# emtiyaz/vmp-for-svae

Measured on AMD Instinct MI355X. Metric: vmp_step_datapoints_per_sec, higher is better.
Workload: dtype f32

## Files before the change

vmp-for-svae_amd/csrc/vmp_mix.hip:

```cpp
#include "vmp_common.h"
#include <stdlib.h>
#include <type_traits>

using namespace vmp;

namespace {

constexpr int TR = 64;
constexpr int LS = 68;
constexpr int MAX_NW = 8;
constexpr int MAX_NW1 = 8;
constexpr int max_nw(int KT) { return KT == 1 ? MAX_NW1 : MAX_NW; }
constexpr int MAX_BLOCKS = 1024;

struct PassArgs {
    const float* x;
    const float* r_in;
    const float* u_in;
    const uint8_t* mask;
    const float* pivot;
    const float* pack;
    float* r_out;
    float* u_out;
    float* logr_out;
    double* partials;
    long long N;
    long long rpw;
    long long rpw_b;
    int K;
    int vec_ok;
    int par_reduce;
#ifdef VMP_DEBUG_TS
    long long* dbg_t;
#endif
};
#ifdef VMP_DEBUG_TS
#define PASS_TS(i) do { if (a.dbg_t && (blockIdx.x == 0 || blockIdx.x == 100) && (threadIdx.x & 63) == 0) { a.dbg_t[(blockIdx.x ? 64 : 0) + (threadIdx.x >> 6) * 8 + (i)] = clock64(); \
    if ((i) == 0 && threadIdx.x == 0) a.dbg_t[(blockIdx.x ? 64 : 0) + 7] = wall_clock64();           \
    if ((i) == 5 && threadIdx.x == 64) a.dbg_t[(blockIdx.x ? 64 : 0) + 8 + 7] = wall_clock64(); } } while (0)
#else
#define PASS_TS(i) do { } while (0)
#endif

template <int D>
__device__ __forceinline__ void load_row(const float* __restrict__ p, float (&o)[D], bool vec) {
    if constexpr (D % 4 == 0) {
        if (vec) {
#pragma unroll
            for (int j = 0; j < D / 4; ++j) {
                float4 v = reinterpret_cast<const float4*>(p)[j];
                o[4 * j] = v.x; o[4 * j + 1] = v.y; o[4 * j + 2] = v.z; o[4 * j + 3] = v.w;
            }
            return;
        }
    } else if constexpr (D % 2 == 0) {
        if (vec) {
#pragma unroll
            for (int j = 0; j < D / 2; ++j) {
                float2 v = reinterpret_cast<const float2*>(p)[j];
                o[2 * j] = v.x; o[2 * j + 1] = v.y;
            }
            return;
        }
    }
#pragma unroll
    for (int j = 0; j < D; ++j) o[j] = p[j];
}

#define VMP_DPP2(OP, CTRL)                                                   \
    "v_" OP "_f32_dpp %0, %0, %0 " CTRL " row_mask:0xf bank_mask:0xf\n\t"  \
    "v_" OP "_f32_dpp %1, %1, %1 " CTRL " row_mask:0xf bank_mask:0xf\n\t"  \
    "s_nop 0\n\t"
#define VMP_DPP2_FIRST(OP, CTRL)                                             \
    "v_" OP "_f32_dpp %0, %2, %2 " CTRL " row_mask:0xf bank_mask:0xf\n\t"  \
    "v_" OP "_f32_dpp %1, %3, %3 " CTRL " row_mask:0xf bank_mask:0xf\n\t"  \
    "s_nop 0\n\t"
__device__ __forceinline__ v2f row16_max2(v2f v) {
    float a, b;
    asm("s_nop 1\n\t" VMP_DPP2_FIRST("max", "row_ror:8") VMP_DPP2("max", "row_ror:4") VMP_DPP2("max", "row_ror:2")
        VMP_DPP2("max", "row_ror:1")
        : "=&v"(a), "=&v"(b) : "v"(v.x), "v"(v.y));
    return v2f{a, b};
}
__device__ __forceinline__ v2f row16_sum2(v2f v) {
    float a, b;
    asm("s_nop 1\n\t" VMP_DPP2_FIRST("add", "row_ror:8") VMP_DPP2("add", "row_ror:4") VMP_DPP2("add", "row_ror:2")
        VMP_DPP2("add", "row_ror:1")
        : "=&v"(a), "=&v"(b) : "v"(v.x), "v"(v.y));
    return v2f{a, b};
}

constexpr int MOM_TERMS = 3;
#ifndef VMP_MOM_FLUSH
#define VMP_MOM_FLUSH 2
#endif

__device__ __forceinline__ double readlane_d(double v, int src_lane) {
    int lo = __double2loint(v), hi = __double2hiint(v);
    lo = __builtin_amdgcn_readlane(lo, src_lane);
    hi = __builtin_amdgcn_readlane(hi, src_lane);
    return __hiloint2double(hi, lo);
}

template <int D, int KT, int FLAV>
__device__ __forceinline__ void pass_epilogue(const PassArgs& a, float* smem, const double (&dacc)[KT][Geo<D>::FT][4],
                                              const double (&dn)[KT][4], int lane, int wave, int nw) {
    using G = Geo<D>;
    constexpr int FT = G::FT;
    constexpr bool SMM = (FLAV == VMP_SMM);
    const int K = a.K;
    {
        __syncthreads();
        PASS_TS(3);
        double* sc = reinterpret_cast<double*>(smem);
        constexpr int SLAB = KT * (FT + 1) * 4 * WAVE;
        if (a.par_reduce) {
            double* mine = sc + wave * SLAB;
#pragma unroll
            for (int kt = 0; kt < KT; ++kt)
#pragma unroll
                for (int c = 0; c < 4; ++c) {
#pragma unroll
                    for (int ft = 0; ft < FT; ++ft) mine[((kt * (FT + 1) + ft) * 4 + c) * WAVE + lane] = dacc[kt][ft][c];
                    mine[((kt * (FT + 1) + FT) * 4 + c) * WAVE + lane] = SMM ? dn[kt][c] : dacc[kt][0][c];
                }
            __syncthreads();
            constexpr int EPT = 2, NWB = max_nw(KT);
            for (int e0 = threadIdx.x; e0 < SLAB; e0 += EPT * blockDim.x) {
                double vals[EPT][NWB];
#pragma unroll
                for (int q = 0; q < EPT; ++q) {
                    const int e = e0 + q * blockDim.x;
#pragma unroll
                    for (int w = 0; w < NWB; ++w) vals[q][w] = (e < SLAB && w < nw) ? sc[w * SLAB + e] : 0.0;
                }
#pragma unroll
                for (int q = 0; q < EPT; ++q) {
                    const int e = e0 + q * blockDim.x;
                    double t2 = vals[q][0];
#pragma unroll
                    for (int w = 1; w < NWB; ++w) t2 += vals[q][w];
                    if (e < SLAB) sc[e] = t2;
                }
            }
            __syncthreads();
        } else {
            for (int w = 0; w < nw; ++w) {
                if (wave == w) {
#pragma unroll
                    for (int kt = 0; kt < KT; ++kt)
#pragma unroll
                        for (int c = 0; c < 4; ++c) {
#pragma unroll
                            for (int ft = 0; ft < FT; ++ft) {
                                const int idx = ((kt * (FT + 1) + ft) * 4 + c) * WAVE + lane;
                                sc[idx] = (w == 0 ? 0.0 : sc[idx]) + dacc[kt][ft][c];
                            }
                            const int idn = ((kt * (FT + 1) + FT) * 4 + c) * WAVE + lane;
                            sc[idn] = (w == 0 ? 0.0 : sc[idn]) + (SMM ? dn[kt][c] : dacc[kt][0][c]);
                        }
                }
                __syncthreads();
            }
        }
        PASS_TS(4);
        constexpr int PX = G::PF + 1;
        double* out = a.partials;
        for (int e = threadIdx.x; e < KT * (FT + 1) * 4 * WAVE; e += blockDim.x) {
            const int l = e & 63, c = (e >> 6) & 3, tf = (e >> 8) % (FT + 1), kt = (e >> 8) / (FT + 1);
            const int k = kt * 16 + (l >> 4) * 4 + c;
            if (k >= K) continue;
            double* row = out + ((long long)k * MAX_BLOCKS + blockIdx.x) * PX;
            if (tf < FT) {
                const int f = tf * 16 + (l & 15);
                if (f < G::F) row[f] = sc[e];
            } else if ((l & 15) == 0) {
                row[G::F] = sc[e];
            }
        }
        if (wave == 0) {
            double ntot = 0.0;
#pragma unroll
            for (int kt = 0; kt < KT; ++kt) {
                const int k = kt * 16 + (lane & 15), l = ((k & 15) >> 2) * 16, c = k & 3;
                const double nk = (lane < 16 && k < K) ? sc[((kt * (FT + 1) + FT) * 4 + c) * WAVE + l] : 0.0;
#pragma unroll
                for (int j = 0; j < 16; ++j) ntot += readlane_d(nk, j);
            }
            for (int k = lane; k < K; k += WAVE) out[((long long)k * MAX_BLOCKS + blockIdx.x) * PX + G::PF] = ntot;
        }
        PASS_TS(5);
    }
}

template <int D, int KT, int FLAV, bool ESTEP, bool STATS, bool MASK>
__global__ __launch_bounds__(max_nw(KT) * WAVE) void pass_kernel(PassArgs a) {
    using G = Geo<D>;
    constexpr int FT = G::FT;
    constexpr bool SMM = (FLAV == VMP_SMM);
    extern __shared__ __attribute__((aligned(16))) float smem[];

    const int lane = threadIdx.x & 63, wave = threadIdx.x >> 6, nw = blockDim.x >> 6;
    const int K = a.K;
    PASS_TS(0);
#ifdef VMP_DEBUG_TS
    if (a.dbg_t && (blockIdx.x == 0 || blockIdx.x == 100) && (threadIdx.x & 63) == 0)
        a.dbg_t[(blockIdx.x ? 64 : 0) + (threadIdx.x >> 6) * 8 + 6] = __builtin_amdgcn_s_getreg((31 << 11) | 4);
#endif
    float* xl = smem + wave * (G::XROWS * LS);
    constexpr int ONE = D, ZERO = D + 1;
    xl[ONE * LS + lane] = 1.0f;
    xl[ZERO * LS + lane] = 0.0f;
    const int ppos = (lane & ~7) + 2 * (lane & 3) + ((lane >> 2) & 1);

    const bool vec = a.vec_ok != 0;
    long long lo, hi;
    if (a.rpw_b == a.rpw) {
        lo = ((long long)blockIdx.x * nw + wave) * a.rpw;
        hi = lo + a.rpw;
    } else {
        const int hw = nw >> 1;
        const long long base = (long long)blockIdx.x * hw * (a.rpw + a.rpw_b);
        lo = wave < hw ? base + wave * a.rpw : base + hw * a.rpw + (wave - hw) * a.rpw_b;
        hi = lo + (wave < hw ? a.rpw : a.rpw_b);
    }
    if (hi > a.N) hi = a.N;
    float xr[D];
    {
        const long long n = lo + lane;
#pragma unroll
        for (int j = 0; j < D; ++j) xr[j] = 0.f;
        if (n < hi) load_row<D>(a.x + n * D, xr, vec);
    }
    const int i16 = lane & 15, kk = lane >> 4;
    float pv[D];
    {
        const float* __restrict__ pp = a.pivot ? a.pivot : a.x;
        const bool hasp = a.pivot != nullptr;
#pragma unroll
        for (int j = 0; j < D; ++j) { const float v = pp[j]; pv[j] = hasp ? v : 0.f; }
    }

    constexpr int MP = (D + 1) / 2, WP = (G::TRI + 1) / 2;
    v2f pm2[KT][MP], pw2[KT][WP], pch[KT];
    float pua[KT], pub[KT];
    if constexpr (ESTEP) {
#pragma unroll
        for (int kt = 0; kt < KT; ++kt) {
            const int k = kt * 16 + i16;
            const bool on = k < K;
            const float* __restrict__ p = a.pack + (on ? k : 0) * G::PACK;
            float raw[G::PACK];
            if (G::PACK % 4 == 0 && (reinterpret_cast<uintptr_t>(a.pack) & 15) == 0) {
#pragma unroll
                for (int j = 0; j < G::PACK / 4; ++j) {
                    const float4 q = reinterpret_cast<const float4*>(p)[j];
                    raw[4 * j] = q.x; raw[4 * j + 1] = q.y; raw[4 * j + 2] = q.z; raw[4 * j + 3] = q.w;
                }
            } else {
#pragma unroll
                for (int j = 0; j < G::PACK; ++j) raw[j] = p[j];
            }
#pragma unroll
            for (int j = 0; j < 2 * MP; ++j) pm2[kt][j >> 1][j & 1] = (on && j < D) ? raw[j < D ? j : 0] - pv[j < D ? j : 0] : 0.f;
#pragma unroll
            for (int j = 0; j < 2 * WP; ++j) pw2[kt][j >> 1][j & 1] = (on && j < G::TRI) ? raw[D + (j < G::TRI ? j : 0)] : 0.f;
            pch[kt].x = on ? raw[D + G::TRI] : -INFINITY;
            pch[kt].y = on ? raw[D + G::TRI + 1] : 0.f;
            pua[kt] = on ? raw[D + G::TRI + 2] : 0.f;
            pub[kt] = on ? raw[D + G::TRI + 3] : 1.f;
        }
    }

    int offA[FT], offB[FT];
#pragma unroll
    for (int ft = 0; ft < FT; ++ft) {
        const int f = ft * 16 + i16;
        int ra = ZERO, rb = ZERO;
        if (f == 0) { ra = ONE; rb = ONE; }
        else if (f <= D) { ra = f - 1; rb = ONE; }
        else if (f < G::F) {
            int p = f - D - 1, d = 0;
            while (p >= D - d) { p -= D - d; ++d; }
            ra = d; rb = d + p;
        }
        offA[ft] = ra * LS + 2 * kk;
        offB[ft] = rb * LS + 2 * kk;
    }

    f32x4 acc[KT][FT], acs[KT][FT];
    f32x4 nacc[KT], nacs[KT];
    double dacc[KT][FT][4];
    double dn[KT][4];
#pragma unroll
    for (int kt = 0; kt < KT; ++kt) {
        nacc[kt] = f32x4{0.f, 0.f, 0.f, 0.f};
        nacs[kt] = f32x4{0.f, 0.f, 0.f, 0.f};
#pragma unroll
        for (int c = 0; c < 4; ++c) dn[kt][c] = 0.0;
#pragma unroll
        for (int ft = 0; ft < FT; ++ft) {
            acc[kt][ft] = f32x4{0.f, 0.f, 0.f, 0.f};
            acs[kt][ft] = f32x4{0.f, 0.f, 0.f, 0.f};
#pragma unroll
            for (int c = 0; c < 4; ++c) dacc[kt][ft][c] = 0.0;
        }
    }

#ifdef VMP_DEBUG_TS
    if (a.dbg_t) {
        float chk = xr[0] + pv[0];
        if constexpr (ESTEP) chk += pm2[0][0][0] + pch[0].x;
        asm volatile("" :: "v"(chk));
        PASS_TS(1);
    }
#endif
    for (long long row0 = lo; row0 < hi; row0 += TR) {
        const int trows = (hi - row0 < TR) ? (int)(hi - row0) : TR;
        {
            const bool valid = row0 + lane < hi;
#pragma unroll
            for (int j = 0; j < D; ++j) xl[j * LS + ppos] = valid ? xr[j] - pv[j] : 0.f;
            const long long n2 = row0 + TR + lane;
#pragma unroll
            for (int j = 0; j < D; ++j) xr[j] = 0.f;
            if (n2 < hi) load_row<D>(a.x + n2 * D, xr, vec);
        }
        __builtin_amdgcn_wave_barrier();

        const long long tbase = (row0 + kk) * K + i16;
        const int K4 = 4 * K;
#pragma unroll 1
        for (int n0 = 0; n0 < trows; n0 += 32) {
            unsigned As[KT][3][4], Rs[KT][3][4], Bs[FT][3][4];
            auto group = [&](auto full_c, auto u_c) __attribute__((always_inline)) {
                constexpr bool FULL = decltype(full_c)::value;
                constexpr int u = decltype(u_c)::value;
                const int n8 = n0 + 8 * u;
// ... 549 lines not shown
                for (int ft = 0; ft < FT; ++ft)
#pragma unroll
                    for (int t = 0; t < 3; ++t)
                        b[ft][t] = __builtin_bit_cast(bf16x8, u32x4{Bs[ft][t][0], Bs[ft][t][1], Bs[ft][t][2], Bs[ft][t][3]});
                bf16x8 av[3];
#pragma unroll
                for (int t = 0; t < 3; ++t) av[t] = __builtin_bit_cast(bf16x8, u32x4{As[t][0], As[t][1], As[t][2], As[t][3]});
#pragma unroll
                for (int ta = 0; ta < MT; ++ta) {
#pragma unroll
                    for (int tb = 0; tb + ta < MT; ++tb) {
#pragma unroll
                        for (int ft = 0; ft < FT; ++ft) {
                            if (ta + tb == 0) acc[0][ft] = __builtin_amdgcn_mfma_f32_16x16x32_bf16(av[ta], b[ft][tb], acc[0][ft], 0, 0, 0);
                            else acs[0][ft] = __builtin_amdgcn_mfma_f32_16x16x32_bf16(av[ta], b[ft][tb], acs[0][ft], 0, 0, 0);
                        }
                    }
                }
            }
            };
            if (full) body(std::integral_constant<bool, true>{});
            else body(std::integral_constant<bool, false>{});
        }

        if constexpr (STATS) {
            if (((row0 - lo) / TR) % VMP_MOM_FLUSH == VMP_MOM_FLUSH - 1 || row0 + TR >= hi) {
#pragma unroll
                for (int c = 0; c < 4; ++c) {
#pragma unroll
                    for (int ft = 0; ft < FT; ++ft) dacc[0][ft][c] += (double)acc[0][ft][c] + (double)acs[0][ft][c];
                }
                if constexpr (SMM) { dnl += (double)nsum; nsum = 0.f; }
#pragma unroll
                for (int ft = 0; ft < FT; ++ft) { acc[0][ft] = f32x4{0.f, 0.f, 0.f, 0.f}; acs[0][ft] = f32x4{0.f, 0.f, 0.f, 0.f}; }
            }
        }
        __builtin_amdgcn_wave_barrier();
    }

    PASS_TS(2);
    if constexpr (STATS && SMM) {
        double tot = dnl;
        {
            int lo = __double2loint(tot), hi = __double2hiint(tot);
            tot += __hiloint2double(__shfl_xor(hi, 32), __shfl_xor(lo, 32));
            lo = __double2loint(tot); hi = __double2hiint(tot);
            tot += __hiloint2double(__shfl_xor(hi, 16), __shfl_xor(lo, 16));
        }
#pragma unroll
        for (int c = 0; c < 4; ++c) {
            const int src = 4 * kk + c;
            const int lo = __shfl(__double2loint(tot), src), hi = __shfl(__double2hiint(tot), src);
            dn[0][c] = __hiloint2double(hi, lo);
        }
    }
    if constexpr (STATS) pass_epilogue<D, 1, FLAV>(a, smem, dacc, dn, lane, wave, nw);
}

template <int D, int FLAV, bool STATS, int MT = 3>
__global__ __launch_bounds__(MAX_NW1 * WAVE) void pass_xdl_kernel(PassArgs a) {
    pass_xdl_body<D, FLAV, STATS, MT>(a);
}

__device__ double digamma_d(double x) {
    double r = 0.0;
    while (x < 10.0) { r -= 1.0 / x; x += 1.0; }
    const double f = 1.0 / (x * x);
    return r + log(x) - 0.5 / x
           - f * (1.0 / 12 - f * (1.0 / 120 - f * (1.0 / 252 - f * (1.0 / 240 - f * (1.0 / 132 - f * (691.0 / 32760))))));
}

template <int D>
__device__ void write_pack(float* pack, int k, const double* m, const double* W ,
                           double c, double h, double ua, double ub) {
    using G = Geo<D>;
    float* p = pack + k * G::PACK;
    int idx = D;
    for (int j = 0; j < D; ++j) p[j] = (float)m[j];
    for (int i = 0; i < D; ++i)
        for (int j = 0; j <= i; ++j) p[idx++] = (float)W[i * D + j];
    const double LOG2E = 1.4426950408889634074;
    p[idx++] = (float)(c * LOG2E); p[idx++] = (float)(h * LOG2E); p[idx++] = (float)ua; p[idx++] = (float)ub;
}

template <int D>
__device__ __forceinline__ bool chol_lower(double (&A)[D * D]) {
    bool ok = true;
#pragma unroll
    for (int j = 0; j < D; ++j) {
        double s = A[j * D + j];
#pragma unroll
        for (int p = 0; p < j; ++p) s -= A[j * D + p] * A[j * D + p];
        ok = ok && (s > 0.0);
        const double d = sqrt(s);
        const double rd = 1.0 / d;
        A[j * D + j] = d;
#pragma unroll
        for (int i = j + 1; i < D; ++i) {
            double t = A[i * D + j];
#pragma unroll
            for (int p = 0; p < j; ++p) t -= A[i * D + p] * A[j * D + p];
            A[i * D + j] = t * rd;
        }
#pragma unroll
        for (int i = 0; i < j; ++i) A[i * D + j] = 0.0;
    }
    return ok;
}

template <int D>
__device__ __forceinline__ void tri_inv_lower(const double (&L)[D * D], double (&Li)[D * D]) {
#pragma unroll
    for (int i = 0; i < D * D; ++i) Li[i] = 0.0;
#pragma unroll
    for (int j = 0; j < D; ++j) {
        Li[j * D + j] = 1.0 / L[j * D + j];
#pragma unroll
        for (int i = j + 1; i < D; ++i) {
            double s = 0.0;
#pragma unroll
            for (int p = j; p < i; ++p) s += L[i * D + p] * Li[p * D + j];
            Li[i * D + j] = -s / L[i * D + i];
        }
    }
}



__device__ __forceinline__ double fast_rsqrt_d(double x) {
    double y = __builtin_amdgcn_rsq(x);
    y = y * (1.5 - 0.5 * x * y * y);
    y = y * (1.5 - 0.5 * x * y * y);
    return y;
}

template <int D>
__device__ __forceinline__ void wave_chol_inverse(const double* A, int lane, double (&X)[D], double& sumlog, bool& ok) {
    double row[D], rd[D];
#pragma unroll
    for (int e = 0; e < D; ++e)
        row[e] = lane < D ? 0.5 * (A[lane * D + e] + A[e * D + lane]) : (e == lane ? 1.0 : 0.0);
    ok = true;
    double mydiag = 1.0;
#pragma unroll
    for (int j = 0; j < D; ++j) {
        double t = row[j];
#pragma unroll
        for (int p = 0; p < j; ++p) t -= row[p] * readlane_d(row[p], j);
        const double sj = readlane_d(t, j);
        ok = ok && (sj > 0.0);
        rd[j] = fast_rsqrt_d(sj);
        if (lane == j) mydiag = sj;
        row[j] = lane >= j ? t * rd[j] : 0.0;
    }
    double lg = lane < D ? 0.5 * log(mydiag) : 0.0;
    sumlog = 0.0;
#pragma unroll
    for (int j = 0; j < D; ++j) sumlog += readlane_d(lg, j);
#pragma unroll
    for (int i = 0; i < D; ++i) {
        double acc = (i == lane) ? 1.0 : 0.0;
#pragma unroll
        for (int p = 0; p < i; ++p) acc -= readlane_d(row[p], i) * X[p];
        X[i] = acc * rd[i];
    }
}

template <int D>
__device__ void estep_constants(int k, int flavour, double alpha_k, double alpha_sum, double beta_k, double v_k,
                                double logdetP, double kap, double& c, double& h, double& ua, double& ub, double& elp) {
    const double LOG2 = 0.69314718055994530942, PI = 3.14159265358979323846;
    elp = digamma_d(alpha_k) - digamma_d(alpha_sum);
    double sdg = 0.0;
    if (flavour == VMP_GMM) {
        for (int i = 0; i < D; ++i) sdg += digamma_d(0.5 * (v_k + 1.0 + i));
        const double ld = (logdetP > log(1e-20)) ? logdetP : 0.0;
        const double eld = sdg + D * LOG2 + ld;
        c = elp + 0.5 * eld - 0.5 * (D / beta_k);
        h = 0.5; ua = 1.0; ub = 1.0;
    } else {
        for (int i = 0; i < D; ++i) sdg += digamma_d(0.5 * (v_k + i));
        const double eld = sdg + D * LOG2 + logdetP;
        h = 0.5 * (D + kap);
        c = lgamma(0.5 * (D + kap)) - lgamma(0.5 * kap) - 0.5 * D * log(kap * PI) + elp + 0.5 * eld
            - h * (D / beta_k) + log(kap);
        ua = D + kap;
        ub = D / beta_k + kap;
    }
}

constexpr int FIN_THREADS = 1024;
constexpr int FIN_MAX_GROUPS = FIN_THREADS / 64;

__device__ __forceinline__ void st_pack(const FinArgs& a, int idx, double v) {
    a.pack[idx] = (float)v;
    if (a.pack64) a.pack64[idx] = v;
}

template <int D>
__device__ void finalize_block(const FinArgs& a, const int k, const int tid, const int nthreads) {
    using G = Geo<D>;
    __shared__ double part[FIN_MAX_GROUPS][64];
    __shared__ double st[G::SW];
    __shared__ double ntot;
    __shared__ double Ck[D * D], mk[D], sp[D + 4], scal[8];
    __shared__ double alpha0s[VMP_MAX_K];
    const int K = a.K;
    const int FIN_GROUPS = nthreads >> 6;
    const bool post = a.do_post != 0;
    const bool smm = a.flavour == VMP_SMM;
    const double beta0 = post ? (double)a.beta0[k] : 0.0, v0 = post ? (double)a.v0[k] : 0.0;
    const double alpha0 = post ? (double)a.alpha0[k] : 0.0;
    const double kap = (post && smm) ? (double)a.kappa[k] : 0.0;
    bool shifted = (a.src == 0) && (a.pivot != nullptr);
    double m0d = 0.0, m0e = 0.0, C0de = 0.0, cd = 0.0, ce = 0.0;
    if (tid < D * D) {
        const int d = tid / D, e = tid % D;
        if (post) { m0d = a.m0[k * D + d]; m0e = a.m0[k * D + e]; C0de = a.C0[(k * D + d) * D + e]; }
        if (shifted) { cd = a.pivot[d]; ce = a.pivot[e]; }
    }
    if (post && tid < K) alpha0s[tid] = a.alpha0[tid];

    FIN_TS(0);
    if (a.src == 0) {
        constexpr int PX = G::PF + 1;
        const int f = tid & 63, g = tid >> 6;
        const double* __restrict__ mine = a.partials + (long long)k * MAX_BLOCKS * PX;
        for (int lg = g; lg < FIN_MAX_GROUPS; lg += FIN_GROUPS) {
            double s = 0.0;
            for (int b0 = lg; b0 < a.nblk; b0 += FIN_MAX_GROUPS * 16) {
                double v1[16];
                const int fc = f < PX ? f : PX - 1;
#pragma unroll
                for (int i = 0; i < 16; ++i) {
                    const int b = b0 + i * FIN_MAX_GROUPS;
                    const int bc = b < a.nblk ? b : a.nblk - 1;
                    v1[i] = mine[(long long)bc * PX + fc];
                }
#pragma unroll
                for (int i = 0; i < 16; ++i) {
                    const bool in = b0 + i * FIN_MAX_GROUPS < a.nblk;
                    v1[i] = (in && f < PX) ? v1[i] : 0.0;
                }
#pragma unroll
                for (int i = 0; i < 16; ++i) s += v1[i];
            }
            part[lg][f] = s;
        }
        __syncthreads();
        FIN_TS(1);
        if (tid < 64) {
            double t1 = 0.0;
            for (int gg = 0; gg < FIN_MAX_GROUPS; ++gg) t1 += part[gg][tid];
            part[0][tid] = t1;
        }
        __syncthreads();
        if (tid == 0) { st[0] = part[0][G::F]; st[1] = part[0][0]; ntot = part[0][G::PF]; }
        if (tid < D) st[2 + tid] = part[0][1 + tid];
        if (tid < D * D) {
            const int d = tid / D, e = tid % D;
            const int lo = d < e ? d : e, hi = d < e ? e : d;
            st[2 + D + tid] = part[0][1 + D + lo * D - lo * (lo - 1) / 2 + (hi - lo)];
        }
    } else {
        for (int i = tid; i < G::SW; i += nthreads) st[i] = a.stats_in[(long long)k * G::SW + i];
        if (tid == 0) {
            double t = 0.0;
            for (int j = 0; j < K; ++j) t += a.stats_in[(long long)j * G::SW];
            ntot = t;
        }
    }
    __syncthreads();
    if (a.nranks >= 1) {
        constexpr int SWP = (G::SW + 1 + 7) & ~7;
        const int par = (int)(a.iter & 1), G_ = a.nranks;
        double val = 0.0;
        if (tid < G::SW) {
            val = st[tid];
            if (shifted && tid >= 2) {
                const double W = st[1];
                if (tid < 2 + D) {
                    val += W * (double)a.pivot[tid - 2];
                } else {
                    const int d = (tid - 2 - D) / D, e = (tid - 2 - D) % D;
                    const double pd = a.pivot[d], pe = a.pivot[e];
                    val += pd * st[2 + e] + st[2 + d] * pe + W * pd * pe;
                }
            }
        } else if (tid == G::SW) {
            val = ntot;
        }
        if (tid <= G::SW) {
            for (int g = 0; g < G_; ++g) {
                double* slot = a.peer[g] + (((size_t)par * G_ + a.rank) * K + k) * SWP;
                __hip_atomic_store(slot + tid, val, __ATOMIC_RELAXED, __HIP_MEMORY_SCOPE_SYSTEM);
            }
            __builtin_amdgcn_fence(__ATOMIC_RELEASE, "");
            asm volatile("s_waitcnt vmcnt(0)" ::: "memory");
        }
        __syncthreads();
        if (tid == 0) {
            __builtin_amdgcn_fence(__ATOMIC_RELEASE, "");
            asm volatile("s_waitcnt vmcnt(0)" ::: "memory");
            for (int g = 0; g < G_; ++g) {
                unsigned long long* fl = reinterpret_cast<unsigned long long*>(a.peer[g] + (size_t)2 * G_ * K * SWP);
                __hip_atomic_store(fl + ((size_t)par * G_ + a.rank) * K + k, a.iter + 1ull, __ATOMIC_RELAXED, __HIP_MEMORY_SCOPE_SYSTEM);
            }
        }
        double* mine = a.peer[a.rank];
        if (tid < G_) {
            const unsigned long long* fl = reinterpret_cast<const unsigned long long*>(mine + (size_t)2 * G_ * K * SWP)
                                           + ((size_t)par * G_ + tid) * K + k;
            const long long t0 = wall_clock64();
            bool ok = false;
            while (!ok) {
                ok = __hip_atomic_load(fl, __ATOMIC_RELAXED, __HIP_MEMORY_SCOPE_SYSTEM) == a.iter + 1ull;
                if (!ok) {
                    if (wall_clock64() - t0 > 400000000ll) break;
                    __builtin_amdgcn_s_sleep(8);
                }
            }
            if (!ok && a.status) *a.status = 1;
        }
        __syncthreads();
        if (tid == 0) __builtin_amdgcn_fence(__ATOMIC_ACQUIRE, "");
        __syncthreads();
        if (tid <= G::SW) {
            double s2 = 0.0;
            for (int g = 0; g < G_; ++g)
                s2 += __hip_atomic_load(mine + (((size_t)par * G_ + g) * K + k) * SWP + tid, __ATOMIC_RELAXED, __HIP_MEMORY_SCOPE_SYSTEM);
            if (tid < G::SW) st[tid] = s2; else ntot = s2;
        }
        shifted = false;
        cd = 0.0; ce = 0.0;
        __syncthreads();
    }
    if (a.stats_out) {
        for (int i = tid; i < G::SW; i += nthreads) {
            double val = st[i];
            if (shifted && i >= 2) {
                const double W = st[1];
                if (i < 2 + D) {
                    val += W * (double)a.pivot[i - 2];
                } else {
                    const int d = (i - 2 - D) / D, e = (i - 2 - D) % D;
                    const double pd = a.pivot[d], pe = a.pivot[e];
                    val += pd * st[2 + e] + st[2 + d] * pe + W * pd * pe;
                }
            }
            a.stats_out[(long long)k * G::SW + i] = val;
        }
    }
    if (!a.do_post) return;

    const double Nk = st[0], Wk = smm ? st[1] : st[0];
    const double* sx = st + 2;
    const double* sxx = st + 2 + D;
    const double den = smm ? (Wk + 1e-20) : Wk;
    const bool empty = (!smm) && !(Wk != 0.0);
    const double alpha_k = alpha0 + Nk;
    const double beta_k = beta0 + Wk;
    const double v_k = smm ? (v0 + Nk) : (v0 + Nk + 1.0);
    FIN_TS(2);
    if (tid < D * D) {
        const int d = tid / D, e = tid % D;
        const double xd = empty ? sx[d] : sx[d] / den, xe = empty ? sx[e] : sx[e] / den;
        const double cen = sxx[d * D + e] - xd * sx[e] - sx[d] * xe + Wk * xd * xe;
        const double Sde = empty ? cen : cen / den;
        const double xrd = empty ? sx[d] + Wk * cd : xd + cd, xre = empty ? sx[e] + Wk * ce : xe + ce;
        const double q0d = xrd - m0d, q0e = xre - m0e;
        const double Cde = C0de + Wk * Sde + (beta0 * Wk / beta_k) * q0d * q0e;
        Ck[d * D + e] = Cde;
        if (a.S) a.S[(k * D + d) * D + e] = (float)Sde;
        if (a.C) a.C[(k * D + d) * D + e] = (float)Cde;
        if (e == 0) {
            const double md = (beta0 * m0d + Wk * xrd) / beta_k;
            mk[d] = md;
            if (a.m) a.m[k * D + d] = (float)md;
            if (a.xbar) a.xbar[k * D + d] = (float)xrd;
        }
    }
    if (tid == 0) {
        if (a.alpha) a.alpha[k] = (float)alpha_k;
        if (a.beta) a.beta[k] = (float)beta_k;
        if (a.v) a.v[k] = (float)v_k;
    }
    __syncthreads();
    FIN_TS(3);
    if (tid < 64) {
        double X[D], sumlog;
        bool ok;
        wave_chol_inverse<D>(Ck, tid, X, sumlog, ok);
        const double sv = ok ? sqrt(v_k) : nan("");
        if (a.pack && tid < D) {
            const int p = k * G::PACK + D;
#pragma unroll
            for (int i = 0; i < D; ++i)
                if (i >= tid) st_pack(a, p + i * (i + 1) / 2 + tid, X[i] * sv);
        }
        if (tid == 0) { scal[0] = -2.0 * sumlog; scal[1] = ok ? 1.0 : 0.0; }
    } else if (tid >= 64 && tid < 64 + D + 2) {
        const int i = tid - 64;
        double arg = 0.5 * (v_k + (smm ? 0.0 : 1.0) + i);
        if (i == D) arg = alpha_k;
        if (i == D + 1) {
            double asum = 0.0;
            for (int j = 0; j < K; ++j) asum += alpha0s[j];
            arg = asum + ntot;
        }
        sp[i] = digamma_d(arg);
    } else if (tid == 128 && smm) {
        sp[D + 2] = lgamma(0.5 * (D + kap)) - lgamma(0.5 * kap);
    }
    __syncthreads();
    FIN_TS(4);
    if (tid == 0) {
        const double LOG2 = 0.69314718055994530942, PI = 3.14159265358979323846;
        const double elp = sp[D] - sp[D + 1];
        double sdg = 0.0;
        for (int i = 0; i < D; ++i) sdg += sp[i];
        double c, h = 0.5, ua = 1.0, ub = 1.0;
        const double logdetP = scal[0];
        if (!smm) {
            const double ld = (logdetP > log(1e-20)) ? logdetP : 0.0;
            c = elp + 0.5 * (sdg + D * LOG2 + ld) - 0.5 * (D / beta_k);
        } else {
            h = 0.5 * (D + kap);
            c = sp[D + 2] - 0.5 * D * log(kap * PI) + elp + 0.5 * (sdg + D * LOG2 + logdetP) - h * (D / beta_k) + log(kap);
            ua = D + kap;
            ub = D / beta_k + kap;
        }
        if (scal[1] == 0.0) c = nan("");
        if (a.pi) a.pi[k] = (float)exp(elp);
        if (a.pack) {
            const int p = k * G::PACK + D + G::TRI;
            const double LOG2E = 1.4426950408889634074;
            st_pack(a, p, c * LOG2E); st_pack(a, p + 1, h * LOG2E); st_pack(a, p + 2, ua); st_pack(a, p + 3, ub);
        }
    }
    if (a.pack && tid < D) st_pack(a, k * G::PACK + tid, mk[tid]);
    FIN_TS(5);
}

template <int D>
__global__ __launch_bounds__(FIN_THREADS) void finalize_kernel(FinArgs a) {
    finalize_block<D>(a, blockIdx.x, threadIdx.x, FIN_THREADS);
}


struct PackArgs {
    int K, flavour;
    const float *alpha, *beta, *m, *P, *v, *kappa;
    float *pack, *pi;
};

template <int D>
__global__ void pack_kernel(PackArgs a) {
    const int k = blockIdx.x * blockDim.x + threadIdx.x;
    if (k >= a.K) return;
    double asum = 0.0;
    for (int j = 0; j < a.K; ++j) asum += a.alpha[j];
    const double v_k = a.v[k];
    double A[D * D], mk[D];
    for (int i = 0; i < D; ++i)
        for (int j = 0; j < D; ++j) {
            const int ri = D - 1 - i, rj = D - 1 - j;
            A[i * D + j] = 0.5 * ((double)a.P[(k * D + ri) * D + rj] + (double)a.P[(k * D + rj) * D + ri]);
        }
    double c = 0, h = 0.5, ua = 1, ub = 1, elp = 0;
    double W[D * D];
    if (chol_lower<D>(A)) {
        double ld = 0.0;
        for (int i = 0; i < D; ++i) ld += log(A[i * D + i]);
        const double sv = sqrt(v_k);
        for (int i = 0; i < D; ++i)
            for (int j = 0; j < D; ++j) W[i * D + j] = sv * A[(D - 1 - j) * D + (D - 1 - i)];
        const double kap = a.flavour == VMP_SMM ? (double)a.kappa[k] : 0.0;
        estep_constants<D>(k, a.flavour, a.alpha[k], asum, a.beta[k], v_k, 2.0 * ld, kap, c, h, ua, ub, elp);
    } else {
        for (int i = 0; i < D * D; ++i) W[i] = nan("");
        c = nan("");
    }
    for (int d = 0; d < D; ++d) mk[d] = a.m[k * D + d];
    if (a.pi) a.pi[k] = (float)exp(elp);
    write_pack<D>(a.pack, k, mk, W, c, h, ua, ub);
}


struct PivotArgs { const float* x; long long N; int D; float* out; };

__global__ __launch_bounds__(1024) void pivot_kernel(PivotArgs a) {
    __shared__ double red[1024];
    const int tid = threadIdx.x;
    const long long S = a.N < 4096 ? a.N : 4096;
    const long long step = a.N / S;
    for (int d = 0; d < a.D; ++d) {
        double s = 0.0;
        for (long long i = tid; i < S; i += 1024) s += (double)a.x[(i * step) * a.D + d];
        red[tid] = s;
        __syncthreads();
        for (int w = 512; w > 0; w >>= 1) {
            if (tid < w) red[tid] += red[tid + w];
            __syncthreads();
        }
        if (tid == 0) a.out[d] = (float)(red[0] / (double)S);
        __syncthreads();
    }
}

__global__ __launch_bounds__(SMALL_STATS_GROUPS * 80) void small_stats_kernel(SmallStatsArgs a) {
    __shared__ double part[SMALL_STATS_GROUPS][80];
    const int SW = 2 + a.D + a.D * a.D, i = threadIdx.x % 80;
    const double t = small_stats_component(a, blockIdx.x, part);
    if (threadIdx.x < 80 && i < SW) a.stats[(long long)blockIdx.x * SW + i] = t;
}

struct Plan {
    int nw, blocks, par_reduce;
    size_t lds;
    long long rpw, rpw_b;
};

Plan make_plan(long long N, int D, int K, int flavour, bool stats, bool xdl = false) {
    Plan p;
    constexpr int tuned_blocks = 256;
    constexpr int tuned_nw = MAX_NW;
    const size_t wreg = (size_t)((D + 2) * LS + (xdl ? TR * AIS : 0)) * sizeof(float);
    int nw = tuned_nw;
    if (nw > max_nw((K + 15) / 16)) nw = max_nw((K + 15) / 16);
    if (nw < 1) nw = 1;
    const long long ntiles = (N + TR - 1) / TR;
    if ((long long)nw > ntiles) nw = (int)ntiles;
    long long blocks = (ntiles + nw - 1) / nw;
    if (blocks > tuned_blocks) blocks = tuned_blocks;
    if (blocks > MAX_BLOCKS) blocks = MAX_BLOCKS;
    long long rpw = (N + blocks * nw - 1) / (blocks * nw);
    rpw = (rpw + 7) / 8 * 8;
    if (rpw < TR) rpw = TR;
    blocks = ((N + rpw - 1) / rpw + nw - 1) / nw;
    p.rpw_b = rpw;
#ifndef VMP_SPLIT_GMM
#define VMP_SPLIT_GMM 64
#endif
#ifndef VMP_SPLIT_SMM
#define VMP_SPLIT_SMM 62
#endif
    const int split = flavour == VMP_SMM ? VMP_SPLIT_SMM : VMP_SPLIT_GMM;
    if (nw == 8 && split != 50 && rpw >= 2 * TR) {
        long long cap = tuned_blocks < MAX_BLOCKS ? tuned_blocks : MAX_BLOCKS;
        long long pr = ((N + 4 * cap - 1) / (4 * cap) + 7) / 8 * 8;
        if (pr < 2 * TR) pr = 2 * TR;
        const long long ra = (pr * split / 100 + 4) / 8 * 8, rb = pr - ra;
        if (rb >= TR) {
            rpw = ra;
            p.rpw_b = rb;
            blocks = (N + 4 * pr - 1) / (4 * pr);
        }
    }
    p.rpw = rpw;
    p.nw = nw;
    p.blocks = (int)blocks;
    const int FTn = (1 + D + D * (D + 1) / 2 + 15) / 16, KTn = (K + 15) / 16;
    const size_t scratch = stats ? (size_t)(KTn <= 2 ? KTn : 4) * (FTn + 1) * 4 * WAVE * sizeof(double) : 0;
    p.lds = wreg * nw;
    p.par_reduce = 0;
    if (scratch * nw <= 64 * 1024) {
        p.par_reduce = 1;
        if (scratch * nw > p.lds) p.lds = scratch * nw;
    } else if (scratch > p.lds) {
        p.lds = scratch;
    }
    return p;
}

template <int D, int KT>
int launch_pass_dk(const PassArgs& a, const Plan& p, int flavour, bool estep, bool stats, bool mask, hipStream_t s) {
    dim3 grid(p.blocks), block(p.nw * WAVE);
#define VMP_LAUNCH(FL, E, S, M) \
    hipLaunchKernelGGL((pass_kernel<D, KT, FL, E, S, M>), grid, block, p.lds, s, a)
    if (flavour == VMP_GMM) {
        if (estep && stats) VMP_LAUNCH(VMP_GMM, true, true, false);
        else if (estep && mask) VMP_LAUNCH(VMP_GMM, true, false, true);
        else if (estep) VMP_LAUNCH(VMP_GMM, true, false, false);
        else VMP_LAUNCH(VMP_GMM, false, true, false);
    } else {
        if (estep && stats) VMP_LAUNCH(VMP_SMM, true, true, false);
        else if (estep) VMP_LAUNCH(VMP_SMM, true, false, false);
        else VMP_LAUNCH(VMP_SMM, false, true, false);
    }
#undef VMP_LAUNCH
    return check_launch("pass_kernel");
}

inline bool use_xdl(int K, bool estep, bool mask) { return estep && !mask && K <= 16; }

#ifndef VMP_MOM2_ROWS
#define VMP_MOM2_ROWS (1ll << 16)
#endif
template <int D>
int launch_pass_xdl(const PassArgs& a, const Plan& p, int flavour, bool stats, hipStream_t s) {
    dim3 grid(p.blocks), block(p.nw * WAVE);
#define VMP_LAUNCH_X(FL, S, M) do { \
        if (p.lds > 64 * 1024) { if (const int rc_ = set_dyn_lds(reinterpret_cast<const void*>(pass_xdl_kernel<D, FL, S, M>), p.lds, "pass_xdl_kernel")) return rc_; } \
        hipLaunchKernelGGL((pass_xdl_kernel<D, FL, S, M>), grid, block, p.lds, s, a); } while (0)
    const bool m2 = stats && a.N >= VMP_MOM2_ROWS;
    if (flavour == VMP_GMM) { if (m2) VMP_LAUNCH_X(VMP_GMM, true, 2); else if (stats) VMP_LAUNCH_X(VMP_GMM, true, 3); else VMP_LAUNCH_X(VMP_GMM, false, 3); }
    else { if (m2) VMP_LAUNCH_X(VMP_SMM, true, 2); else if (stats) VMP_LAUNCH_X(VMP_SMM, true, 3); else VMP_LAUNCH_X(VMP_SMM, false, 3); }
#undef VMP_LAUNCH_X
    return check_launch("pass_xdl_kernel");
}

template <int D>
int launch_pass_d(const PassArgs& a, const Plan& p, int flavour, bool estep, bool stats, bool mask, hipStream_t s) {
    if (use_xdl(a.K, estep, mask)) return launch_pass_xdl<D>(a, p, flavour, stats, s);
    const int KT = (a.K + 15) / 16;
    if (KT == 1) return launch_pass_dk<D, 1>(a, p, flavour, estep, stats, mask, s);
    if (KT == 2) return launch_pass_dk<D, 2>(a, p, flavour, estep, stats, mask, s);
    return launch_pass_dk<D, 4>(a, p, flavour, estep, stats, mask, s);
}

#define VMP_DISPATCH_D(D, CALL)            \
    switch (D) {                            \
        case 1: { constexpr int DD = 1; CALL; } break; \
        case 2: { constexpr int DD = 2; CALL; } break; \
        case 3: { constexpr int DD = 3; CALL; } break; \
        case 4: { constexpr int DD = 4; CALL; } break; \
        case 5: { constexpr int DD = 5; CALL; } break; \
        case 6: { constexpr int DD = 6; CALL; } break; \
        case 7: { constexpr int DD = 7; CALL; } break; \
        case 8: { constexpr int DD = 8; CALL; } break; \
        default: break;                     \
    }

int check_dims(int64_t N, int D, int K) {
    if (N <= 0) { set_error("N must be positive (got %lld)", (long long)N); return VMP_E_BADARG; }
    if (D < 1 || D > VMP_MAX_D) { set_error("D=%d outside compiled range 1..%d", D, VMP_MAX_D); return VMP_E_DIM; }
    if (K < 1 || K > VMP_MAX_K) { set_error("K=%d outside compiled range 1..%d", K, VMP_MAX_K); return VMP_E_DIM; }
    return 0;
}

bool aligned16(const void* p) { return (reinterpret_cast<uintptr_t>(p) & 15) == 0; }

#ifdef VMP_DEBUG_TS
static long long* g_dbg_pass = nullptr;
static long long* g_dbg_t = nullptr;
#endif
int run_pass(PassArgs a, int D, int flavour, bool estep, bool stats, bool mask, hipStream_t s) {
    Plan p = make_plan(a.N, D, a.K, flavour, stats, use_xdl(a.K, estep, mask));
    a.rpw = p.rpw;
    a.rpw_b = p.rpw_b;
    a.par_reduce = p.par_reduce;
#ifdef VMP_DEBUG_TS
    a.dbg_t = g_dbg_pass;
#endif

    int rc = -1;
    VMP_DISPATCH_D(D, rc = launch_pass_d<DD>(a, p, flavour, estep, stats, mask, s));
    return rc;
}

int run_finalize(FinArgs f, int D, hipStream_t s) {
    int rc = -1;
#ifdef VMP_DEBUG_TS
    f.dbg_t = g_dbg_t;
#endif

    VMP_DISPATCH_D(D, {
        hipLaunchKernelGGL((finalize_kernel<DD>), dim3(f.K), dim3(FIN_THREADS), 0, s, f);
        rc = check_launch("finalize_kernel");
    });
    return rc;
}

struct AccArgs { const float* x; const double* pack; float* r; float* u; float* logr; long long N; int K; };
template <int D, bool SMM>
__global__ __launch_bounds__(256) void estep_f64_kernel(AccArgs a) {
    using G = Geo<D>;
    extern __shared__ double spk[];
    for (int e = threadIdx.x; e < a.K * G::PACK; e += blockDim.x) spk[e] = a.pack[e];
    __syncthreads();
    const double LN2 = 0.69314718055994530942;
    for (long long n = (long long)blockIdx.x * blockDim.x + threadIdx.x; n < a.N; n += (long long)gridDim.x * blockDim.x) {
        double xd[D];
#pragma unroll
        for (int j = 0; j < D; ++j) xd[j] = (double)a.x[n * D + j];
        auto quad = [&](int k) {
            const double* __restrict__ p = spk + k * G::PACK;
            double q = 0.0;
#pragma unroll
            for (int i = 0; i < D; ++i) {
                double y = 0.0;
#pragma unroll
                for (int j = 0; j <= i; ++j) y = fma(p[D + i * (i + 1) / 2 + j], xd[j] - p[j], y);
                q = fma(y, y, q);
            }
            return q;
        };
        double mx = -INFINITY;
        for (int k = 0; k < a.K; ++k) {
            const double* __restrict__ p = spk + k * G::PACK;
            const double l2 = p[D + G::TRI] - p[D + G::TRI + 1] * quad(k);
            mx = l2 > mx ? l2 : mx;
        }
        double ssum = 0.0;
        for (int k = 0; k < a.K; ++k) {
            const double* __restrict__ p = spk + k * G::PACK;
            ssum += exp2(p[D + G::TRI] - p[D + G::TRI + 1] * quad(k) - mx);
        }
        const double inv = 1.0 / ssum, l2s = log2(ssum);
        for (int k = 0; k < a.K; ++k) {
            const double* __restrict__ p = spk + k * G::PACK;
            const double q = quad(k);
            const double l2 = p[D + G::TRI] - p[D + G::TRI + 1] * q - mx;
            a.r[n * a.K + k] = (float)(exp2(l2) * inv);
            if (a.logr) a.logr[n * a.K + k] = (float)((l2 - l2s) * LN2);
            if constexpr (SMM) a.u[n * a.K + k] = (float)(p[D + G::TRI + 2] / (q + p[D + G::TRI + 3]));
        }
    }
}

constexpr int ACC_RS = 128, ACC_THREADS = 1024, ACC_ITEMS = 3;
struct AccStatArgs { const float *x, *r, *u, *pivot; double* partials; long long N, rows_per_block; int K; };
template <int D>
__global__ __launch_bounds__(ACC_THREADS) void stats_f64_kernel(AccStatArgs a) {
    using G = Geo<D>;
    constexpr int FP = G::F + 1;
    constexpr int XS = D + 1;
    extern __shared__ float sm[];
    const int K = a.K;
    float* xs = sm;
    float* ws_ = sm + ACC_RS * XS;
    float* us_ = ws_ + ACC_RS * K;
// ... 331 lines not shown
```

Measured before the change: 20.81 billion.

## Fuse pass epilogue reduction with partial emission and trim finalize barriers

The pass epilogue now writes each reduced element straight to the global partials buffer inside the cross-wave reduction loop. This removes one block barrier and a second pass over shared memory, and per-component counts are saved to a small extra LDS array. In finalize, the Cholesky triangular solve is folded into the factorization loop and several block-wide __syncthreads are replaced with wave-level barriers or register broadcasts via readlane. The digamma and scalar setup is also spread across threads. The change adds LDS sizing for the count array and a dynamic-LDS opt-in when the allocation exceeds 64KB, at the cost of more complex synchronisation reasoning.

```diff
diff --git a/vmp-for-svae_amd/csrc/vmp_mix.hip b/vmp-for-svae_amd/csrc/vmp_mix.hip
--- a/vmp-for-svae_amd/csrc/vmp_mix.hip
+++ b/vmp-for-svae_amd/csrc/vmp_mix.hip
@@ -114,6 +114,22 @@
         PASS_TS(3);
         double* sc = reinterpret_cast<double*>(smem);
         constexpr int SLAB = KT * (FT + 1) * 4 * WAVE;
+        double* nks = sc + (a.par_reduce ? nw : 1) * SLAB;
+        constexpr int PX = G::PF + 1;
+        double* out = a.partials;
+        auto emit = [&](int e, double val) __attribute__((always_inline)) {
+            const int l = e & 63, c = (e >> 6) & 3, tf = (e >> 8) % (FT + 1), kt = (e >> 8) / (FT + 1);
+            const int k = kt * 16 + (l >> 4) * 4 + c;
+            if (k >= K) return;
+            double* row = out + ((long long)k * MAX_BLOCKS + blockIdx.x) * PX;
+            if (tf < FT) {
+                const int f = tf * 16 + (l & 15);
+                if (f < G::F) row[f] = val;
+            } else if ((l & 15) == 0) {
+                row[G::F] = val;
+                nks[k] = val;
+            }
+        };
         if (a.par_reduce) {
             double* mine = sc + wave * SLAB;
 #pragma unroll
@@ -140,10 +156,9 @@
                     double t2 = vals[q][0];
 #pragma unroll
                     for (int w = 1; w < NWB; ++w) t2 += vals[q][w];
-                    if (e < SLAB) sc[e] = t2;
-                }
-            }
-            __syncthreads();
+                    if (e < SLAB) emit(e, t2);
+                }
+            }
         } else {
             for (int w = 0; w < nw; ++w) {
                 if (wave == w) {
@@ -162,28 +177,16 @@
                 }
                 __syncthreads();
             }
-        }
+            for (int e = threadIdx.x; e < SLAB; e += blockDim.x) emit(e, sc[e]);
+        }
+        __syncthreads();
         PASS_TS(4);
-        constexpr int PX = G::PF + 1;
-        double* out = a.partials;
-        for (int e = threadIdx.x; e < KT * (FT + 1) * 4 * WAVE; e += blockDim.x) {
-            const int l = e & 63, c = (e >> 6) & 3, tf = (e >> 8) % (FT + 1), kt = (e >> 8) / (FT + 1);
-            const int k = kt * 16 + (l >> 4) * 4 + c;
-            if (k >= K) continue;
-            double* row = out + ((long long)k * MAX_BLOCKS + blockIdx.x) * PX;
-            if (tf < FT) {
-                const int f = tf * 16 + (l & 15);
-                if (f < G::F) row[f] = sc[e];
-            } else if ((l & 15) == 0) {
-                row[G::F] = sc[e];
-            }
-        }
         if (wave == 0) {
             double ntot = 0.0;
 #pragma unroll
             for (int kt = 0; kt < KT; ++kt) {
-                const int k = kt * 16 + (lane & 15), l = ((k & 15) >> 2) * 16, c = k & 3;
-                const double nk = (lane < 16 && k < K) ? sc[((kt * (FT + 1) + FT) * 4 + c) * WAVE + l] : 0.0;
+                const int k = kt * 16 + (lane & 15);
+                const double nk = (lane < 16 && k < K) ? nks[k] : 0.0;
 #pragma unroll
                 for (int j = 0; j < 16; ++j) ntot += readlane_d(nk, j);
             }
@@ -1039,18 +1042,15 @@
         rd[j] = fast_rsqrt_d(sj);
         if (lane == j) mydiag = sj;
         row[j] = lane >= j ? t * rd[j] : 0.0;
+        double acc = (j == lane) ? 1.0 : 0.0;
+#pragma unroll
+        for (int p = 0; p < j; ++p) acc -= readlane_d(row[p], j) * X[p];
+        X[j] = acc * rd[j];
     }
     double lg = lane < D ? 0.5 * log(mydiag) : 0.0;
     sumlog = 0.0;
 #pragma unroll
     for (int j = 0; j < D; ++j) sumlog += readlane_d(lg, j);
-#pragma unroll
-    for (int i = 0; i < D; ++i) {
-        double acc = (i == lane) ? 1.0 : 0.0;
-#pragma unroll
-        for (int p = 0; p < i; ++p) acc -= readlane_d(row[p], i) * X[p];
-        X[i] = acc * rd[i];
-    }
 }
 
 template <int D>
@@ -1084,13 +1084,19 @@
     if (a.pack64) a.pack64[idx] = v;
 }
 
+__device__ __forceinline__ void wave_lds_sync() {
+    __builtin_amdgcn_fence(__ATOMIC_RELEASE, "wavefront");
+    __builtin_amdgcn_wave_barrier();
+    __builtin_amdgcn_fence(__ATOMIC_ACQUIRE, "wavefront");
+}
+
 template <int D>
 __device__ void finalize_block(const FinArgs& a, const int k, const int tid, const int nthreads) {
     using G = Geo<D>;
     __shared__ double part[FIN_MAX_GROUPS][64];
     __shared__ double st[G::SW];
     __shared__ double ntot;
-    __shared__ double Ck[D * D], mk[D], sp[D + 4], scal[8];
+    __shared__ double Ck[D * D], scal[8];
     __shared__ double alpha0s[VMP_MAX_K];
     const int K = a.K;
     const int FIN_GROUPS = nthreads >> 6;
@@ -1107,6 +1113,8 @@
         if (shifted) { cd = a.pivot[d]; ce = a.pivot[e]; }
     }
     if (post && tid < K) alpha0s[tid] = a.alpha0[tid];
+    const bool fast = post && a.src == 0 && a.nranks < 1 && !a.stats_out;
+    double sN = 0.0, sW = 0.0, sT = 0.0;
 
     FIN_TS(0);
     if (a.src == 0) {
@@ -1136,18 +1144,23 @@
         }
         __syncthreads();
         FIN_TS(1);
+        auto gsum = [&](int f_) { double t1 = 0.0; for (int gg = 0; gg < FIN_MAX_GROUPS; ++gg) t1 += part[gg][f_]; return t1; };
         if (tid < 64) {
-            double t1 = 0.0;
-            for (int gg = 0; gg < FIN_MAX_GROUPS; ++gg) t1 += part[gg][tid];
-            part[0][tid] = t1;
-        }
-        __syncthreads();
-        if (tid == 0) { st[0] = part[0][G::F]; st[1] = part[0][0]; ntot = part[0][G::PF]; }
-        if (tid < D) st[2 + tid] = part[0][1 + tid];
-        if (tid < D * D) {
-            const int d = tid / D, e = tid % D;
-            const int lo = d < e ? d : e, hi = d < e ? e : d;
-            st[2 + D + tid] = part[0][1 + D + lo * D - lo * (lo - 1) / 2 + (hi - lo)];
+            const double t1 = gsum(tid);
+            if (tid == G::F) st[0] = t1;
+            if (tid == 0) st[1] = t1;
+            if (tid == G::PF) ntot = t1;
+            if (tid >= 1 && tid <= D) st[2 + tid - 1] = t1;
+            if (tid > D && tid < G::F) {
+                int p = tid - D - 1, lo = 0;
+                while (p >= D - lo) { p -= D - lo; ++lo; }
+                const int hi = lo + p;
+                st[2 + D + lo * D + hi] = t1;
+                st[2 + D + hi * D + lo] = t1;
+            }
+            sN = readlane_d(t1, G::F); sW = readlane_d(t1, 0); sT = readlane_d(t1, G::PF);
+        } else if (fast && tid < 192) {
+            sN = gsum(G::F); sW = gsum(0); sT = gsum(G::PF);
         }
     } else {
         for (int i = tid; i < G::SW; i += nthreads) st[i] = a.stats_in[(long long)k * G::SW + i];
@@ -1157,7 +1170,8 @@
             ntot = t;
         }
     }
-    __syncthreads();
+    if (fast) wave_lds_sync();
+    else __syncthreads();
     if (a.nranks >= 1) {
         constexpr int SWP = (G::SW + 1 + 7) & ~7;
         const int par = (int)(a.iter & 1), G_ = a.nranks;
@@ -1240,7 +1254,8 @@
     }
     if (!a.do_post) return;
 
-    const double Nk = st[0], Wk = smm ? st[1] : st[0];
+    if (!fast) { sN = st[0]; sW = st[1]; sT = ntot; }
+    const double Nk = sN, Wk = smm ? sW : sN;
     const double* sx = st + 2;
     const double* sxx = st + 2 + D;
     const double den = smm ? (Wk + 1e-20) : Wk;
@@ -1249,36 +1264,37 @@
     const double beta_k = beta0 + Wk;
     const double v_k = smm ? (v0 + Nk) : (v0 + Nk + 1.0);
     FIN_TS(2);
-    if (tid < D * D) {
-        const int d = tid / D, e = tid % D;
-        const double xd = empty ? sx[d] : sx[d] / den, xe = empty ? sx[e] : sx[e] / den;
-        const double cen = sxx[d * D + e] - xd * sx[e] - sx[d] * xe + Wk * xd * xe;
-        const double Sde = empty ? cen : cen / den;
-        const double xrd = empty ? sx[d] + Wk * cd : xd + cd, xre = empty ? sx[e] + Wk * ce : xe + ce;
-        const double q0d = xrd - m0d, q0e = xre - m0e;
-        const double Cde = C0de + Wk * Sde + (beta0 * Wk / beta_k) * q0d * q0e;
-        Ck[d * D + e] = Cde;
-        if (a.S) a.S[(k * D + d) * D + e] = (float)Sde;
-        if (a.C) a.C[(k * D + d) * D + e] = (float)Cde;
-        if (e == 0) {
-            const double md = (beta0 * m0d + Wk * xrd) / beta_k;
-            mk[d] = md;
-            if (a.m) a.m[k * D + d] = (float)md;
-            if (a.xbar) a.xbar[k * D + d] = (float)xrd;
-        }
-    }
-    if (tid == 0) {
-        if (a.alpha) a.alpha[k] = (float)alpha_k;
-        if (a.beta) a.beta[k] = (float)beta_k;
-        if (a.v) a.v[k] = (float)v_k;
-    }
-    __syncthreads();
-    FIN_TS(3);
     if (tid < 64) {
+        if (tid < D * D) {
+            const int d = tid / D, e = tid % D;
+            const double xd = empty ? sx[d] : sx[d] / den, xe = empty ? sx[e] : sx[e] / den;
+            const double cen = sxx[d * D + e] - xd * sx[e] - sx[d] * xe + Wk * xd * xe;
+            const double Sde = empty ? cen : cen / den;
+            const double xrd = empty ? sx[d] + Wk * cd : xd + cd, xre = empty ? sx[e] + Wk * ce : xe + ce;
+            const double q0d = xrd - m0d, q0e = xre - m0e;
+            const double Cde = C0de + Wk * Sde + (beta0 * Wk / beta_k) * q0d * q0e;
+            Ck[d * D + e] = Cde;
+            if (a.S) a.S[(k * D + d) * D + e] = (float)Sde;
+            if (a.C) a.C[(k * D + d) * D + e] = (float)Cde;
+            if (e == 0) {
+                const double md = (beta0 * m0d + Wk * xrd) / beta_k;
+                if (a.m) a.m[k * D + d] = (float)md;
+                if (a.xbar) a.xbar[k * D + d] = (float)xrd;
+                if (a.pack) st_pack(a, k * G::PACK + d, md);
+            }
+        }
+        if (tid == 0) {
+            if (a.alpha) a.alpha[k] = (float)alpha_k;
+            if (a.beta) a.beta[k] = (float)beta_k;
+            if (a.v) a.v[k] = (float)v_k;
+        }
+        wave_lds_sync();
+        FIN_TS(3);
+        const double svk = sqrt(v_k);
         double X[D], sumlog;
         bool ok;
         wave_chol_inverse<D>(Ck, tid, X, sumlog, ok);
-        const double sv = ok ? sqrt(v_k) : nan("");
+        const double sv = ok ? svk : nan("");
         if (a.pack && tid < D) {
             const int p = k * G::PACK + D;
 #pragma unroll
@@ -1286,46 +1302,51 @@
                 if (i >= tid) st_pack(a, p + i * (i + 1) / 2 + tid, X[i] * sv);
         }
         if (tid == 0) { scal[0] = -2.0 * sumlog; scal[1] = ok ? 1.0 : 0.0; }
-    } else if (tid >= 64 && tid < 64 + D + 2) {
+    } else if (tid < 128) {
         const int i = tid - 64;
         double arg = 0.5 * (v_k + (smm ? 0.0 : 1.0) + i);
         if (i == D) arg = alpha_k;
         if (i == D + 1) {
             double asum = 0.0;
             for (int j = 0; j < K; ++j) asum += alpha0s[j];
-            arg = asum + ntot;
-        }
-        sp[i] = digamma_d(arg);
-    } else if (tid == 128 && smm) {
-        sp[D + 2] = lgamma(0.5 * (D + kap)) - lgamma(0.5 * kap);
+            arg = asum + sT;
+        }
+        if (i > D + 1) arg = 16.0;
+        const double dg = digamma_d(arg);
+        double sdg = 0.0;
+#pragma unroll
+        for (int j = 0; j < D; ++j) sdg += readlane_d(dg, j);
+        const double elp = readlane_d(dg, D) - readlane_d(dg, D + 1);
+        if (i == 0) {
+            scal[2] = elp; scal[3] = sdg;
+            if (a.pi) a.pi[k] = (float)exp(elp);
+        }
+    } else if (tid == 128) {
+        const double PI = 3.14159265358979323846;
+        scal[4] = D / beta_k;
+        if (smm) { scal[5] = lgamma(0.5 * (D + kap)) - lgamma(0.5 * kap); scal[6] = log(kap * PI); scal[7] = log(kap); }
     }
     __syncthreads();
     FIN_TS(4);
-    if (tid == 0) {
-        const double LOG2 = 0.69314718055994530942, PI = 3.14159265358979323846;
-        const double elp = sp[D] - sp[D + 1];
-        double sdg = 0.0;
-        for (int i = 0; i < D; ++i) sdg += sp[i];
+    if (tid == 0 && a.pack) {
+        const double LOG2 = 0.69314718055994530942;
+        const double elp = scal[2], sdg = scal[3], hb = scal[4];
         double c, h = 0.5, ua = 1.0, ub = 1.0;
         const double logdetP = scal[0];
         if (!smm) {
             const double ld = (logdetP > log(1e-20)) ? logdetP : 0.0;
-            c = elp + 0.5 * (sdg + D * LOG2 + ld) - 0.5 * (D / beta_k);
+            c = elp + 0.5 * (sdg + D * LOG2 + ld) - 0.5 * hb;
         } else {
             h = 0.5 * (D + kap);
-            c = sp[D + 2] - 0.5 * D * log(kap * PI) + elp + 0.5 * (sdg + D * LOG2 + logdetP) - h * (D / beta_k) + log(kap);
+            c = scal[5] - 0.5 * D * scal[6] + elp + 0.5 * (sdg + D * LOG2 + logdetP) - h * hb + scal[7];
             ua = D + kap;
-            ub = D / beta_k + kap;
+            ub = hb + kap;
         }
         if (scal[1] == 0.0) c = nan("");
-        if (a.pi) a.pi[k] = (float)exp(elp);
-        if (a.pack) {
-            const int p = k * G::PACK + D + G::TRI;
-            const double LOG2E = 1.4426950408889634074;
-            st_pack(a, p, c * LOG2E); st_pack(a, p + 1, h * LOG2E); st_pack(a, p + 2, ua); st_pack(a, p + 3, ub);
-        }
-    }
-    if (a.pack && tid < D) st_pack(a, k * G::PACK + tid, mk[tid]);
+        const int p = k * G::PACK + D + G::TRI;
+        const double LOG2E = 1.4426950408889634074;
+        st_pack(a, p, c * LOG2E); st_pack(a, p + 1, h * LOG2E); st_pack(a, p + 2, ua); st_pack(a, p + 3, ub);
+    }
     FIN_TS(5);
 }
 
@@ -1449,13 +1470,14 @@
     p.blocks = (int)blocks;
     const int FTn = (1 + D + D * (D + 1) / 2 + 15) / 16, KTn = (K + 15) / 16;
     const size_t scratch = stats ? (size_t)(KTn <= 2 ? KTn : 4) * (FTn + 1) * 4 * WAVE * sizeof(double) : 0;
+    const size_t nkb = stats ? (size_t)(KTn <= 2 ? KTn : 4) * 16 * sizeof(double) : 0;
     p.lds = wreg * nw;
     p.par_reduce = 0;
     if (scratch * nw <= 64 * 1024) {
         p.par_reduce = 1;
-        if (scratch * nw > p.lds) p.lds = scratch * nw;
-    } else if (scratch > p.lds) {
-        p.lds = scratch;
+        if (scratch * nw + nkb > p.lds) p.lds = scratch * nw + nkb;
+    } else if (scratch + nkb > p.lds) {
+        p.lds = scratch + nkb;
     }
     return p;
 }
@@ -1463,8 +1485,9 @@
 template <int D, int KT>
 int launch_pass_dk(const PassArgs& a, const Plan& p, int flavour, bool estep, bool stats, bool mask, hipStream_t s) {
     dim3 grid(p.blocks), block(p.nw * WAVE);
-#define VMP_LAUNCH(FL, E, S, M) \
-    hipLaunchKernelGGL((pass_kernel<D, KT, FL, E, S, M>), grid, block, p.lds, s, a)
+#define VMP_LAUNCH(FL, E, S, M) do { \
+        if (p.lds > 64 * 1024) { if (const int rc_ = set_dyn_lds(reinterpret_cast<const void*>(pass_kernel<D, KT, FL, E, S, M>), p.lds, "pass_kernel")) return rc_; } \
+        hipLaunchKernelGGL((pass_kernel<D, KT, FL, E, S, M>), grid, block, p.lds, s, a); } while (0)
     if (flavour == VMP_GMM) {
         if (estep && stats) VMP_LAUNCH(VMP_GMM, true, true, false);
         else if (estep && mask) VMP_LAUNCH(VMP_GMM, true, false, true);
```

New measurement: 20.91 billion, median of 6. About the same (+0.5%).
